# TinfoilHat0/Defending-Against-Backdoors-with-Robust-Learning-Rate

Hardware: NVIDIA H100
Metric: fl_rounds_per_sec (higher is better)
Workload: dtype bf16

## Files before the change

defending-against-backdoors-with-robust-learning-rate_b200/ops/csrc/common.cuh:

```cuda
#pragma once
#include <cuda_runtime.h>
#include <cuda_bf16.h>
#include <stdint.h>

#include "dropspec.h"

#define RLR_CUDA_CHECK(expr)                                                                     \
    do {                                                                                         \
        cudaError_t _e = (expr);                                                                 \
        if (_e != cudaSuccess) return _e;                                                        \
    } while (0)

namespace rlr {

constexpr int kWarp = 32;

__device__ __forceinline__ void pdl_wait() { asm volatile("griddepcontrol.wait;" ::: "memory"); }
__device__ __forceinline__ void pdl_trigger() { asm volatile("griddepcontrol.launch_dependents;" ::: "memory"); }

extern int g_pdl;
bool pdl_enabled();

template <typename... KArgs, typename... Args>
inline cudaError_t launch_kernel(void (*kernel)(KArgs...), dim3 grid, dim3 block, size_t smem, cudaStream_t st, Args&&... args) {
    if (!pdl_enabled()) {
        kernel<<<grid, block, smem, st>>>(static_cast<KArgs>(args)...);
        return cudaGetLastError();
    }
    cudaLaunchConfig_t cfg = {};
    cfg.gridDim = grid; cfg.blockDim = block; cfg.dynamicSmemBytes = smem; cfg.stream = st;
    cudaLaunchAttribute attr[1];
    attr[0].id = cudaLaunchAttributeProgrammaticStreamSerialization;
    attr[0].val.programmaticStreamSerializationAllowed = 1;
    cfg.attrs = attr; cfg.numAttrs = 1;
    return cudaLaunchKernelEx(&cfg, kernel, static_cast<KArgs>(args)...);
}

void* scratch_alloc(size_t bytes, cudaStream_t st);
void scratch_free(void* p);
struct Scratch {
    void* p;
    Scratch(size_t bytes, cudaStream_t st) : p(scratch_alloc(bytes, st)) {}
    ~Scratch() { scratch_free(p); }
    Scratch(const Scratch&) = delete;
    Scratch& operator=(const Scratch&) = delete;
    template <typename T> T* as() const { return static_cast<T*>(p); }
};
template <typename T>
__global__ void __launch_bounds__(256) ordered_sum_kernel(T* __restrict__ out, const T* __restrict__ part, int nparts, long long n) {
    pdl_wait();
    pdl_trigger();
    for (long long i = (long long)blockIdx.x * 256 + threadIdx.x; i < n; i += (long long)gridDim.x * 256) {
        T s = part[i];
        for (int j = 1; j < nparts; ++j) s += part[(size_t)j * n + i];
        out[i] += s;
    }
}

template <typename T>
__global__ void __launch_bounds__(256) ordered_sum_cols_kernel(T* __restrict__ out, const T* __restrict__ part, int nparts, long long n) {
    constexpr int kRows = 64, kPerWarp = kRows / 8;
    __shared__ T tile[kRows][33];
    pdl_wait();
    pdl_trigger();
    const int lane = threadIdx.x & 31, warp = threadIdx.x >> 5;
    const long long col = (long long)blockIdx.x * 32 + lane;
    T s = T(0);
    for (int j0 = 0; j0 < nparts; j0 += kRows) {
        T v[kPerWarp];
#pragma unroll
        for (int q = 0; q < kPerWarp; ++q) {
            const int j = j0 + warp + 8 * q;
            v[q] = (j < nparts && col < n) ? part[(size_t)j * n + col] : T(0);
        }
#pragma unroll
        for (int q = 0; q < kPerWarp; ++q) tile[warp + 8 * q][lane] = v[q];
        __syncthreads();
        if (warp == 0) {
            const int rows = nparts - j0 < kRows ? nparts - j0 : kRows;
            int r = 0;
            if (j0 == 0) { s = tile[0][lane]; r = 1; }
            for (; r < rows; ++r) s += tile[r][lane];
        }
        __syncthreads();
    }
    if (warp == 0 && col < n) out[col] += s;
}

__device__ __forceinline__ unsigned long long gtimer() {
    unsigned long long t;
    asm volatile("mov.u64 %0, %%globaltimer;" : "=l"(t));
    return t;
}

__device__ __forceinline__ float warp_sum(float v) {
#pragma unroll
    for (int o = 16; o > 0; o >>= 1) v += __shfl_xor_sync(0xffffffffu, v, o);
    return v;
}
__device__ __forceinline__ double warp_sum(double v) {
#pragma unroll
    for (int o = 16; o > 0; o >>= 1) v += __shfl_xor_sync(0xffffffffu, v, o);
    return v;
}
__device__ __forceinline__ unsigned long long warp_sum(unsigned long long v) {
#pragma unroll
    for (int o = 16; o > 0; o >>= 1) v += __shfl_xor_sync(0xffffffffu, v, o);
    return v;
}
__device__ __forceinline__ int warp_sum(int v) {
#pragma unroll
    for (int o = 16; o > 0; o >>= 1) v += __shfl_xor_sync(0xffffffffu, v, o);
    return v;
}

__device__ __forceinline__ float warp_transpose_sum32(float (&v)[32], int lane) {
#define RLR_TSTAGE(O, N)                                                         \
    {                                                                            \
        const bool up = (lane & (O)) != 0;                                       \
        _Pragma("unroll") for (int i = 0; i < (N); ++i) {                        \
            const float send = up ? v[i] : v[i + (N)];                           \
            const float keep = up ? v[i + (N)] : v[i];                           \
            v[i] = keep + __shfl_xor_sync(0xffffffffu, send, (O));               \
        }                                                                        \
    }
    RLR_TSTAGE(16, 16) RLR_TSTAGE(8, 8) RLR_TSTAGE(4, 4) RLR_TSTAGE(2, 2) RLR_TSTAGE(1, 1)
#undef RLR_TSTAGE
    return v[0];
}

template <typename T>
__device__ __forceinline__ T block_sum(T v, T* scratch) {
    v = warp_sum(v);
    const int lane = threadIdx.x & 31, wid = threadIdx.x >> 5;
    if (lane == 0) scratch[wid] = v;
    __syncthreads();
    const int nw = (blockDim.x + 31) >> 5;
    v = (threadIdx.x < nw) ? scratch[threadIdx.x] : T(0);
    if (wid == 0) v = warp_sum(v);
    __syncthreads();
    return v;
}

__device__ __forceinline__ float4 ld_stream_f4(const float* p) {
    float4 r;
    asm volatile("ld.global.nc.L1::no_allocate.v4.f32 {%0,%1,%2,%3}, [%4];"
                 : "=f"(r.x), "=f"(r.y), "=f"(r.z), "=f"(r.w) : "l"(p));
    return r;
}
__device__ __forceinline__ float4 ld_f4(const float* p) {
    float4 r;
    asm volatile("ld.global.v4.f32 {%0,%1,%2,%3}, [%4];"
                 : "=f"(r.x), "=f"(r.y), "=f"(r.z), "=f"(r.w) : "l"(p));
    return r;
}
__device__ __forceinline__ float ld_f1(const float* p) {
    float r;
    asm volatile("ld.global.f32 %0, [%1];" : "=f"(r) : "l"(p));
    return r;
}
__device__ __forceinline__ void st_f4(float* p, float4 v) {
    asm volatile("st.global.v4.f32 [%0], {%1,%2,%3,%4};" ::"l"(p), "f"(v.x), "f"(v.y), "f"(v.z), "f"(v.w) : "memory");
}
__device__ __forceinline__ void multimem_st_f4(float* mc, float4 v) {
    asm volatile("multimem.st.relaxed.sys.global.v4.f32 [%0], {%1,%2,%3,%4};" ::"l"(mc), "f"(v.x), "f"(v.y),
                 "f"(v.z), "f"(v.w) : "memory");
}
__device__ __forceinline__ void multimem_st_b2(uint2* mc, uint2 v) {
    asm volatile("multimem.st.relaxed.sys.global.v2.f32 [%0], {%1,%2};" ::"l"(mc), "f"(__uint_as_float(v.x)),
                 "f"(__uint_as_float(v.y)) : "memory");
}

__device__ __forceinline__ void st_release_sys(uint32_t* p, uint32_t v) {
    asm volatile("st.release.sys.global.u32 [%0], %1;" ::"l"(p), "r"(v) : "memory");
}
__device__ __forceinline__ uint32_t ld_acquire_sys(const uint32_t* p) {
    uint32_t v;
    asm volatile("ld.acquire.sys.global.u32 %0, [%1];" : "=r"(v) : "l"(p) : "memory");
    return v;
}
__device__ __forceinline__ void st_release_gpu(uint32_t* p, uint32_t v) {
    asm volatile("st.release.gpu.global.u32 [%0], %1;" ::"l"(p), "r"(v) : "memory");
}
__device__ __forceinline__ uint32_t ld_acquire_gpu(const uint32_t* p) {
    uint32_t v;
    asm volatile("ld.acquire.gpu.global.u32 %0, [%1];" : "=r"(v) : "l"(p) : "memory");
    return v;
}

struct Philox {
    uint32_t k0, k1;
    __device__ __forceinline__ Philox(uint64_t seed) : k0((uint32_t)seed), k1((uint32_t)(seed >> 32)) {}
    __device__ __forceinline__ uint4 operator()(uint64_t ctr, uint64_t stream) const {
        uint32_t c0 = (uint32_t)ctr, c1 = (uint32_t)(ctr >> 32), c2 = (uint32_t)stream, c3 = (uint32_t)(stream >> 32);
        uint32_t a = k0, b = k1;
#pragma unroll
        for (int r = 0; r < 10; ++r) {
            const uint32_t hi0 = __umulhi(0xD2511F53u, c0), lo0 = 0xD2511F53u * c0;
            const uint32_t hi1 = __umulhi(0xCD9E8D57u, c2), lo1 = 0xCD9E8D57u * c2;
            const uint32_t n0 = hi1 ^ c1 ^ a, n2 = hi0 ^ c3 ^ b;
            c0 = n0; c1 = lo1; c2 = n2; c3 = lo0;
            a += 0x9E3779B9u; b += 0xBB67AE85u;
        }
        return make_uint4(c0, c1, c2, c3);
    }
};
__device__ __forceinline__ float u32_to_unit(uint32_t x) {
    return ((float)(x >> 8) + 1.0f) * (1.0f / 16777216.0f);
}
__device__ __forceinline__ float4 philox_normal4(const Philox& ph, uint64_t ctr, uint64_t stream) {
    const uint4 u = ph(ctr, stream);
    const float r0 = sqrtf(-2.0f * logf(u32_to_unit(u.x))), r1 = sqrtf(-2.0f * logf(u32_to_unit(u.z)));
    float s0, c0, s1, c1;
    sincospif(2.0f * u32_to_unit(u.y), &s0, &c0);
    sincospif(2.0f * u32_to_unit(u.w), &s1, &c1);
    return make_float4(r0 * c0, r0 * s0, r1 * c1, r1 * s1);
}

__device__ __forceinline__ uint32_t dropout_keep8(const DropSpec& d, long long q) {
    const Philox ph(d.seed);
    const uint4 u = ph((uint64_t)q, ((uint64_t)(*d.step) << 20) ^ d.stream);
    const uint32_t r[4] = {u.x, u.y, u.z, u.w};
    uint32_t keep = 0;
#pragma unroll
    for (int i = 0; i < 8; ++i) keep |= (uint32_t)(((r[i >> 1] >> (16 * (i & 1))) & 0xffffu) >= d.thr) << i;
    return keep;
}

template <typename T>
inline cudaError_t launch_ordered_sum(T* out, const T* part, int nparts, long long n, cudaStream_t st) {
    if (nparts >= 16)
        return launch_kernel(ordered_sum_cols_kernel<T>, dim3((unsigned)((n + 31) / 32)), dim3(256), (size_t)0, st, out, part, nparts, n);
    long long blocks = (n + 255) / 256;
    if (blocks > 1024) blocks = 1024;
    if (blocks < 1) blocks = 1;
    return launch_kernel(ordered_sum_kernel<T>, dim3((unsigned)blocks), dim3(256), (size_t)0, st, out, part, nparts, n);
}

__device__ __forceinline__ uint32_t pack_bf16x2(float lo, float hi) {
    __nv_bfloat162 v = __floats2bfloat162_rn(lo, hi);
    return *reinterpret_cast<uint32_t*>(&v);
}

}
```

defending-against-backdoors-with-robust-learning-rate_b200/ops/csrc/norm.cu:

```cuda
#include <stdlib.h>

#include "common.cuh"
#include "gemm.h"

namespace rlr {

struct bf8 { float v[8]; };
__device__ __forceinline__ bf8 load8(const __nv_bfloat16* p) {
    const uint4 u = *reinterpret_cast<const uint4*>(p);
    const __nv_bfloat162* h = reinterpret_cast<const __nv_bfloat162*>(&u);
    bf8 r;
#pragma unroll
    for (int i = 0; i < 4; ++i) { const float2 f = __bfloat1622float2(h[i]); r.v[2 * i] = f.x; r.v[2 * i + 1] = f.y; }
    return r;
}
__device__ __forceinline__ void store8(__nv_bfloat16* p, const bf8& r) {
    uint4 u;
    u.x = pack_bf16x2(r.v[0], r.v[1]); u.y = pack_bf16x2(r.v[2], r.v[3]);
    u.z = pack_bf16x2(r.v[4], r.v[5]); u.w = pack_bf16x2(r.v[6], r.v[7]);
    *reinterpret_cast<uint4*>(p) = u;
}
static inline int rows_grid(long long M, int rows_per_block, int num_sms, int per_sm) {
    long long want = (M + rows_per_block - 1) / rows_per_block;
    long long cap = (long long)num_sms * per_sm;
    return (int)(want < 1 ? 1 : (want > cap ? cap : want));
}
static inline bool chan_ok(int C) { return C >= 8 && C <= 2048 && (C % 8) == 0 && (256 % (C / 8)) == 0; }

template <int MODE, bool kRecompute = false>
__global__ void __launch_bounds__(256, MODE == 0 ? 4 : 3) channel_reduce_kernel(const __nv_bfloat16* __restrict__ x, const __nv_bfloat16* __restrict__ dy,
                                                               const __nv_bfloat16* __restrict__ y, const float* __restrict__ mean_rstd,
                                                               float* __restrict__ part , long long M, int C, int relu,
                                                               const float* __restrict__ gamma = nullptr, const float* __restrict__ beta = nullptr,
                                                               int out_cols = 0 ) {
    extern __shared__ float sh[];
    pdl_wait();
    pdl_trigger();
    const int tpr = C / 8, rpi = 256 / tpr;
    const int cg = threadIdx.x % tpr, ry = threadIdx.x / tpr;
    float a[8], b[8], mu[8], rs[8], msc[8], msh[8];
#pragma unroll
    for (int i = 0; i < 8; ++i) { a[i] = 0.f; b[i] = 0.f; mu[i] = 0.f; rs[i] = 1.f; msc[i] = 0.f; msh[i] = 1.f; }
    if (MODE == 1) {
#pragma unroll
        for (int i = 0; i < 8; ++i) { mu[i] = mean_rstd[cg * 8 + i]; rs[i] = mean_rstd[C + cg * 8 + i]; }
        if (kRecompute) {
#pragma unroll
            for (int i = 0; i < 8; ++i) { msc[i] = gamma[cg * 8 + i] * rs[i]; msh[i] = beta[cg * 8 + i] - mu[i] * msc[i]; }
        }
    }
    constexpr int U = MODE == 0 ? 4 : 2;
    const long long stride = (long long)gridDim.x * rpi;
    for (long long r0 = (long long)blockIdx.x * rpi + ry; r0 < M; r0 += stride * U) {
        uint4 xr[U], dr[U], yr[U];
#pragma unroll
        for (int u = 0; u < U; ++u) {
            const long long r = r0 + u * stride;
            const size_t off = (size_t)(r < M ? r : r0) * C + cg * 8;
            xr[u] = *reinterpret_cast<const uint4*>(x + off);
            if (MODE == 1) {
                dr[u] = *reinterpret_cast<const uint4*>(dy + off);
                if (!kRecompute && relu) yr[u] = *reinterpret_cast<const uint4*>(y + off);
            }
        }
#pragma unroll
        for (int u = 0; u < U; ++u) {
            if (r0 + u * stride >= M) continue;
            const __nv_bfloat162* xh = reinterpret_cast<const __nv_bfloat162*>(&xr[u]);
            const __nv_bfloat162* dh = reinterpret_cast<const __nv_bfloat162*>(&dr[u]);
            const __nv_bfloat162* yh = reinterpret_cast<const __nv_bfloat162*>(&yr[u]);
#pragma unroll
            for (int i = 0; i < 4; ++i) {
                const float2 xv = __bfloat1622float2(xh[i]);
                if (MODE == 0) {
                    a[2 * i] += xv.x; a[2 * i + 1] += xv.y; b[2 * i] += xv.x * xv.x; b[2 * i + 1] += xv.y * xv.y;
                } else {
                    float2 dz = __bfloat1622float2(dh[i]);
                    if (!kRecompute && relu) {
                        const float2 yv = __bfloat1622float2(yh[i]);
                        dz.x = yv.x > 0.f ? dz.x : 0.f; dz.y = yv.y > 0.f ? dz.y : 0.f;
                    } else if (kRecompute) {
                        dz.x = (xv.x * msc[2 * i] + msh[2 * i]) > 0.f ? dz.x : 0.f;
                        dz.y = (xv.y * msc[2 * i + 1] + msh[2 * i + 1]) > 0.f ? dz.y : 0.f;
                    }
                    a[2 * i] += dz.x; a[2 * i + 1] += dz.y;
                    b[2 * i] += dz.x * (xv.x - mu[2 * i]) * rs[2 * i]; b[2 * i + 1] += dz.y * (xv.y - mu[2 * i + 1]) * rs[2 * i + 1];
                }
            }
        }
    }
    float* mine = sh + (size_t)ry * 2 * C + cg * 8;
#pragma unroll
    for (int i = 0; i < 8; ++i) { mine[i] = a[i]; mine[C + i] = b[i]; }
    __syncthreads();
    const int ncols = out_cols > 0 ? out_cols : 2 * C;
    float* dst = part + (size_t)blockIdx.x * ncols;
    for (int i = threadIdx.x; i < ncols; i += 256) {
        float t = 0.f;
        for (int r = 0; r < rpi; ++r) t += sh[(size_t)r * 2 * C + i];
        dst[i] = t;
    }
}

cudaError_t launch_ordered_sum_f32(float* out, const float* part, int nparts, long long n, cudaStream_t st) {
    return launch_ordered_sum(out, part, nparts, n, st);
}
cudaError_t launch_ordered_sum_f64(double* out, const double* part, int nparts, long long n, cudaStream_t st) {
    return launch_ordered_sum(out, part, nparts, n, st);
}

cudaError_t launch_channel_stats(const __nv_bfloat16* x, long long M, int C, float* stats, int num_sms, cudaStream_t st, int only_sum, int nslots) {
    if (!chan_ok(C) || nslots < 1) return cudaErrorInvalidValue;
    const int rpi = 256 / (C / 8);
    const int grid = rows_grid(M, rpi * 8, num_sms, nslots >= 4 ? 4 : 2), ncols = only_sum ? C : 2 * C;
    Scratch part((size_t)grid * ncols * sizeof(float), st);
    RLR_CUDA_CHECK(launch_kernel(channel_reduce_kernel<0, false>, dim3(grid), dim3(256), (size_t)rpi * 2 * C * sizeof(float), st, x, nullptr,
                                 nullptr, nullptr, part.as<float>(), M, C, 0, nullptr, nullptr, only_sum ? C : 0));
    return launch_ordered_sum(stats, part.as<float>(), grid, (long long)ncols, st);
}
cudaError_t launch_bn_bwd_reduce(const __nv_bfloat16* dy, const __nv_bfloat16* y, const __nv_bfloat16* x, const float* mean_rstd,
                                 float* dsum, long long M, int C, int relu, int num_sms, cudaStream_t st, const float* gamma,
                                 const float* beta, int nslots) {
    if (!chan_ok(C) || (relu == 2 && (!gamma || !beta)) || (relu == 1 && !y) || nslots < 1) return cudaErrorInvalidValue;
    const int rpi = 256 / (C / 8);
    const int grid = rows_grid(M, rpi * 8, num_sms, nslots >= 3 ? 3 : 2);
    const size_t smem = (size_t)rpi * 2 * C * sizeof(float);
    Scratch part((size_t)grid * 2 * C * sizeof(float), st);
    if (relu == 2)
        RLR_CUDA_CHECK(launch_kernel(channel_reduce_kernel<1, true>, dim3(grid), dim3(256), smem, st, x, dy, y, mean_rstd, part.as<float>(), M, C,
                                     relu, gamma, beta, 0));
    else
        RLR_CUDA_CHECK(launch_kernel(channel_reduce_kernel<1, false>, dim3(grid), dim3(256), smem, st, x, dy, y, mean_rstd, part.as<float>(), M, C,
                                     relu, nullptr, nullptr, 0));
    return launch_ordered_sum(dsum, part.as<float>(), grid, 2LL * C, st);
}

__global__ void bn_finalize_kernel(const float* __restrict__ stats, int slots, float* __restrict__ mean_rstd, float* running_mean,
                                   float* running_var, int C, float count, float eps, float momentum, int train) {
    const int c = blockIdx.x * blockDim.x + threadIdx.x;
    if (c >= C) return;
    if (train) {
        float s1 = 0.f, s2 = 0.f;
        for (int k = 0; k < slots; ++k) { s1 += stats[(size_t)k * 2 * C + c]; s2 += stats[(size_t)k * 2 * C + C + c]; }
        const float mean = s1 / count;
        const float var = fmaxf(s2 / count - mean * mean, 0.f);
        mean_rstd[c] = mean;
        mean_rstd[C + c] = rsqrtf(var + eps);
        running_mean[c] = (1.f - momentum) * running_mean[c] + momentum * mean;
        const float unbiased = count > 1.f ? var * count / (count - 1.f) : var;
        running_var[c] = (1.f - momentum) * running_var[c] + momentum * unbiased;
    } else {
        mean_rstd[c] = running_mean[c];
        mean_rstd[C + c] = rsqrtf(running_var[c] + eps);
    }
}
cudaError_t launch_bn_finalize(const float* stats, int slots, float* mean_rstd, float* running_mean, float* running_var, int C,
                               float count, float eps, float momentum, int train, cudaStream_t st) {
    bn_finalize_kernel<<<(C + 127) / 128, 128, 0, st>>>(stats, slots, mean_rstd, running_mean, running_var, C, count, eps, momentum, train);
    return cudaGetLastError();
}

struct BnFinalize {
    int mode;
    const float* stats; int slots;
    float count, eps, momentum;
    float* running_mean; float* running_var;
};
template <int U, int kMinBlocks>
__global__ void __launch_bounds__(256, kMinBlocks) bn_apply_kernel(const __nv_bfloat16* __restrict__ x, const __nv_bfloat16* __restrict__ res,
                                                         __nv_bfloat16* __restrict__ y, const float* __restrict__ gamma,
                                                         const float* __restrict__ beta, float* __restrict__ mean_rstd,
                                                         long long M, int C, int relu, BnFinalize fin) {
    pdl_wait();
    pdl_trigger();
    const int tpr = C / 8, rpi = 256 / tpr;
    const int cg = threadIdx.x % tpr, ry = threadIdx.x / tpr;
    float sc[8], sh[8];
#pragma unroll
    for (int i = 0; i < 8; ++i) {
        const int c = cg * 8 + i;
        float mean, rstd;
        if (fin.mode == 1) {
            float s1 = 0.f, s2 = 0.f;
            for (int k = 0; k < fin.slots; ++k) { s1 += fin.stats[(size_t)k * 2 * C + c]; s2 += fin.stats[(size_t)k * 2 * C + C + c]; }
            mean = s1 / fin.count;
            const float var = fmaxf(s2 / fin.count - mean * mean, 0.f);
            rstd = rsqrtf(var + fin.eps);
            if (blockIdx.x == 0 && ry == 0) {
                mean_rstd[c] = mean; mean_rstd[C + c] = rstd;
                fin.running_mean[c] = (1.f - fin.momentum) * fin.running_mean[c] + fin.momentum * mean;
                const float unbiased = fin.count > 1.f ? var * fin.count / (fin.count - 1.f) : var;
                fin.running_var[c] = (1.f - fin.momentum) * fin.running_var[c] + fin.momentum * unbiased;
            }
        } else if (fin.mode == 2) {
            mean = fin.running_mean[c]; rstd = rsqrtf(fin.running_var[c] + fin.eps);
        } else {
            mean = mean_rstd[c]; rstd = mean_rstd[C + c];
        }
        sc[i] = gamma[c] * rstd;
        sh[i] = beta[c] - mean * sc[i];
    }
    const long long stride = (long long)gridDim.x * rpi;
    for (long long r0 = (long long)blockIdx.x * rpi + ry; r0 < M; r0 += stride * U) {
        uint4 xr[U], rr[U];
#pragma unroll
        for (int u = 0; u < U; ++u) {
            const long long r = r0 + u * stride;
            const size_t off = (size_t)(r < M ? r : r0) * C + cg * 8;
            xr[u] = *reinterpret_cast<const uint4*>(x + off);
            if (res) rr[u] = *reinterpret_cast<const uint4*>(res + off);
        }
#pragma unroll
        for (int u = 0; u < U; ++u) {
            const long long r = r0 + u * stride;
            if (r >= M) continue;
            const __nv_bfloat162* xh = reinterpret_cast<const __nv_bfloat162*>(&xr[u]);
            const __nv_bfloat162* rh = reinterpret_cast<const __nv_bfloat162*>(&rr[u]);
            bf8 v;
#pragma unroll
            for (int i = 0; i < 4; ++i) {
                const float2 xv = __bfloat1622float2(xh[i]);
                v.v[2 * i] = xv.x * sc[2 * i] + sh[2 * i]; v.v[2 * i + 1] = xv.y * sc[2 * i + 1] + sh[2 * i + 1];
                if (res) { const float2 q = __bfloat1622float2(rh[i]); v.v[2 * i] += q.x; v.v[2 * i + 1] += q.y; }
                if (relu) { v.v[2 * i] = fmaxf(v.v[2 * i], 0.f); v.v[2 * i + 1] = fmaxf(v.v[2 * i + 1], 0.f); }
            }
            store8(y + (size_t)r * C + cg * 8, v);
        }
    }
}
cudaError_t launch_bn_apply(const __nv_bfloat16* x, const __nv_bfloat16* res, __nv_bfloat16* y, const float* gamma, const float* beta,
                            float* mean_rstd, long long M, int C, int relu, int fin_mode, const float* stats, int slots, float count,
                            float eps, float momentum, float* running_mean, float* running_var, int num_sms, cudaStream_t st) {
    if (!chan_ok(C)) return cudaErrorInvalidValue;
    const int rpi = 256 / (C / 8);
    BnFinalize fin{fin_mode, stats, slots, count, eps, momentum, running_mean, running_var};
    static const int unroll = [] { const char* e = getenv("RLR_BN_UNROLL"); return e ? atoi(e) : 1; }();
    static const int occ = [] { const char* e = getenv("RLR_BN_OCC"); return e ? atoi(e) : 0; }();
    if (unroll <= 1 && occ)
        return launch_kernel(bn_apply_kernel<1, 6>, dim3(rows_grid(M, rpi * 4, num_sms, 12)), dim3(256), (size_t)0, st, x, res, y, gamma, beta, mean_rstd,
                             M, C, relu, fin);
    if (unroll <= 1)
        return launch_kernel(bn_apply_kernel<1, 1>, dim3(rows_grid(M, rpi * 4, num_sms, 8)), dim3(256), (size_t)0, st, x, res, y, gamma, beta, mean_rstd, M,
                             C, relu, fin);
    return launch_kernel(bn_apply_kernel<4, 1>, dim3(rows_grid(M, rpi * 4, num_sms, 6)), dim3(256), (size_t)0, st, x, res, y, gamma, beta, mean_rstd, M, C,
                         relu, fin);
}

template <bool kRecompute, int U, int kMinBlocks = 1>
__global__ void __launch_bounds__(256, kMinBlocks) bn_bwd_apply_kernel(const __nv_bfloat16* __restrict__ dy, const __nv_bfloat16* __restrict__ y,
                                                             const __nv_bfloat16* __restrict__ x, const float* __restrict__ gamma,
                                                             const float* __restrict__ mean_rstd, const float* __restrict__ dsum,
                                                             __nv_bfloat16* __restrict__ dx, __nv_bfloat16* __restrict__ dres,
                                                             float* dgamma, float* dbeta, long long M, int C, int relu,
                                                             const float* __restrict__ beta = nullptr, int nslots = 1) {
    pdl_wait();
    pdl_trigger();
    const int tpr = C / 8, rpi = 256 / tpr;
    const int cg = threadIdx.x % tpr, ry = threadIdx.x / tpr;
    float mu[8], rs[8], g[8], k1[8], k2[8], msh[8];
    const float invM = 1.0f / (float)M;
#pragma unroll
    for (int i = 0; i < 8; ++i) {
        const int c = cg * 8 + i;
        mu[i] = mean_rstd[c]; rs[i] = mean_rstd[C + c]; g[i] = gamma[c] * rs[i];
        float s0 = 0.f, s1 = 0.f;
        for (int k = 0; k < nslots; ++k) { s0 += dsum[(size_t)k * 2 * C + c]; s1 += dsum[(size_t)k * 2 * C + C + c]; }
        k1[i] = s0 * invM; k2[i] = s1 * invM;
        msh[i] = kRecompute ? beta[c] - mu[i] * g[i] : 0.f;
    }
    if (blockIdx.x == 0 && ry == 0) {
#pragma unroll
        for (int i = 0; i < 8; ++i) { dbeta[cg * 8 + i] = k1[i] * (float)M; dgamma[cg * 8 + i] = k2[i] * (float)M; }
    }
    const long long stride = (long long)gridDim.x * rpi;
    for (long long r0 = (long long)blockIdx.x * rpi + ry; r0 < M; r0 += stride * U) {
        bf8 dzv[U], xvv[U], yvv[U];
#pragma unroll
        for (int u = 0; u < U; ++u) {
            const long long r = r0 + u * stride;
            const size_t off = (size_t)(r < M ? r : r0) * C + cg * 8;
            dzv[u] = load8(dy + off);
            xvv[u] = load8(x + off);
            if (!kRecompute && relu) yvv[u] = load8(y + off);
        }
#pragma unroll
        for (int u = 0; u < U; ++u) {
            const long long r = r0 + u * stride;
            if (r >= M) continue;
            const size_t off = (size_t)r * C + cg * 8;
            bf8 dz = dzv[u];
            const bf8 xv = xvv[u];
            if (!kRecompute && relu) {
#pragma unroll
                for (int i = 0; i < 8; ++i) dz.v[i] = yvv[u].v[i] > 0.f ? dz.v[i] : 0.f;
            } else if (kRecompute) {
#pragma unroll
                for (int i = 0; i < 8; ++i) dz.v[i] = (xv.v[i] * g[i] + msh[i]) > 0.f ? dz.v[i] : 0.f;
            }
            if (dres) store8(dres + off, dz);
            bf8 o;
#pragma unroll
            for (int i = 0; i < 8; ++i) o.v[i] = g[i] * (dz.v[i] - k1[i] - (xv.v[i] - mu[i]) * rs[i] * k2[i]);
            store8(dx + off, o);
        }
    }
}
cudaError_t launch_bn_bwd_apply(const __nv_bfloat16* dy, const __nv_bfloat16* y, const __nv_bfloat16* x, const float* gamma,
                                const float* mean_rstd, const float* dsum, __nv_bfloat16* dx, __nv_bfloat16* dres, float* dgamma,
                                float* dbeta, long long M, int C, int relu, int num_sms, cudaStream_t st, const float* beta, int nslots) {
    if (!chan_ok(C) || (relu == 2 && !beta) || (relu == 1 && !y) || nslots < 1) return cudaErrorInvalidValue;
    const int rpi = 256 / (C / 8);
    const int grid = rows_grid(M, rpi * 4, num_sms, 8);
    static const int unroll = [] { const char* e = getenv("RLR_BN_UNROLL"); return e ? atoi(e) : 1; }();
    if (unroll > 1) {
        if (relu == 2)
            return launch_kernel(bn_bwd_apply_kernel<true, 2>, dim3(grid), dim3(256), (size_t)0, st, dy, y, x, gamma, mean_rstd, dsum, dx, dres, dgamma,
                                 dbeta, M, C, relu, beta, nslots);
        return launch_kernel(bn_bwd_apply_kernel<false, 2>, dim3(grid), dim3(256), (size_t)0, st, dy, y, x, gamma, mean_rstd, dsum, dx, dres, dgamma, dbeta,
                             M, C, relu, nullptr, nslots);
    }
    static const int occ = [] { const char* e = getenv("RLR_BN_OCC"); return e ? atoi(e) : 0; }();
    if (occ) {
        const int grid2 = rows_grid(M, rpi * 4, num_sms, 12);
        if (relu == 2)
            return launch_kernel(bn_bwd_apply_kernel<true, 1, 4>, dim3(grid2), dim3(256), (size_t)0, st, dy, y, x, gamma, mean_rstd, dsum, dx, dres, dgamma,
                                 dbeta, M, C, relu, beta, nslots);
        return launch_kernel(bn_bwd_apply_kernel<false, 1, 4>, dim3(grid2), dim3(256), (size_t)0, st, dy, y, x, gamma, mean_rstd, dsum, dx, dres, dgamma,
                             dbeta, M, C, relu, nullptr, nslots);
    }
    if (relu == 2)
        return launch_kernel(bn_bwd_apply_kernel<true, 1>, dim3(grid), dim3(256), (size_t)0, st, dy, y, x, gamma, mean_rstd, dsum, dx, dres, dgamma, dbeta, M,
                             C, relu, beta, nslots);
    return launch_kernel(bn_bwd_apply_kernel<false, 1>, dim3(grid), dim3(256), (size_t)0, st, dy, y, x, gamma, mean_rstd, dsum, dx, dres, dgamma, dbeta, M, C,
                         relu, nullptr, nslots);
}

__global__ void __launch_bounds__(256) relu_bwd_kernel(__nv_bfloat16* __restrict__ dy, const __nv_bfloat16* __restrict__ y, long long n8, float scale) {
    for (long long q = (long long)blockIdx.x * blockDim.x + threadIdx.x; q < n8; q += (long long)gridDim.x * blockDim.x) {
        bf8 d = load8(dy + 8 * q);
        const bf8 yv = load8(y + 8 * q);
#pragma unroll
        for (int i = 0; i < 8; ++i) d.v[i] = yv.v[i] > 0.f ? d.v[i] * scale : 0.f;
        store8(dy + 8 * q, d);
    }
}
cudaError_t launch_relu_bwd(__nv_bfloat16* dy, const __nv_bfloat16* y, long long n, int num_sms, cudaStream_t st, float scale) {
    if (n % 8) return cudaErrorInvalidValue;
    relu_bwd_kernel<<<rows_grid(n / 8, 256, num_sms, 8), 256, 0, st>>>(dy, y, n / 8, scale);
    return cudaGetLastError();
}

__global__ void __launch_bounds__(256) maxpool2_fwd_kernel(const __nv_bfloat16* __restrict__ x, __nv_bfloat16* __restrict__ y,
                                                             uint8_t* __restrict__ idx, int B, int H, int W, int C, DropSpec drop) {
    const int Ho = H / 2, Wo = W / 2, cg_n = C / 8;
    const long long total = (long long)B * Ho * Wo * cg_n;
    for (long long t = (long long)blockIdx.x * blockDim.x + threadIdx.x; t < total; t += (long long)gridDim.x * blockDim.x) {
        const int cg = (int)(t % cg_n);
        long long r = t / cg_n;
        const int wo = (int)(r % Wo); r /= Wo;
        const int ho = (int)(r % Ho);
        const int b = (int)(r / Ho);
        const __nv_bfloat16* base = x + (((size_t)b * H + 2 * ho) * W + 2 * wo) * C + cg * 8;
        bf8 best = load8(base);
        uint8_t bi[8] = {0, 0, 0, 0, 0, 0, 0, 0};
#pragma unroll
        for (int k = 1; k < 4; ++k) {
            const bf8 v = load8(base + ((size_t)(k >> 1) * W + (k & 1)) * C);
#pragma unroll
            for (int i = 0; i < 8; ++i) if (v.v[i] > best.v[i]) { best.v[i] = v.v[i]; bi[i] = (uint8_t)k; }
        }
        const size_t o = (((size_t)b * Ho + ho) * Wo + wo) * C + cg * 8;
        if (drop.thr) {
            const uint32_t keep = dropout_keep8(drop, (long long)(o >> 3));
#pragma unroll
            for (int i = 0; i < 8; ++i) best.v[i] = (keep >> i & 1) ? best.v[i] * drop.scale : 0.f;
        }
        store8(y + o, best);
        uint2 pk;
        pk.x = bi[0] | (bi[1] << 8) | (bi[2] << 16) | (bi[3] << 24);
        pk.y = bi[4] | (bi[5] << 8) | (bi[6] << 16) | (bi[7] << 24);
        *reinterpret_cast<uint2*>(idx + o) = pk;
    }
}
__global__ void __launch_bounds__(256) maxpool2_bwd_kernel(const __nv_bfloat16* __restrict__ dy, const uint8_t* __restrict__ idx,
                                                             __nv_bfloat16* __restrict__ dx, const __nv_bfloat16* __restrict__ zmask,
                                                             int B, int H, int W, int C, DropSpec drop) {
    const int Ho = H / 2, Wo = W / 2, cg_n = C / 8;
    const long long total = (long long)B * Ho * Wo * cg_n;
    for (long long t = (long long)blockIdx.x * blockDim.x + threadIdx.x; t < total; t += (long long)gridDim.x * blockDim.x) {
        const int cg = (int)(t % cg_n);
        long long r = t / cg_n;
        const int wo = (int)(r % Wo); r /= Wo;
        const int ho = (int)(r % Ho);
        const int b = (int)(r / Ho);
        const size_t src = (size_t)t * 8;
        bf8 g = load8(dy + src);
        if (drop.thr) {
            const uint32_t keep = dropout_keep8(drop, (long long)(src >> 3));
#pragma unroll
            for (int i = 0; i < 8; ++i) g.v[i] = (keep >> i & 1) ? g.v[i] * drop.scale : 0.f;
        }
        if (zmask) {
            const bf8 z = load8(zmask + src);
#pragma unroll
            for (int i = 0; i < 8; ++i) g.v[i] = z.v[i] > 0.f ? g.v[i] : 0.f;
        }
        const uint2 pk = *reinterpret_cast<const uint2*>(idx + src);
        bf8 zero;
#pragma unroll
        for (int i = 0; i < 8; ++i) zero.v[i] = 0.f;
#pragma unroll
        for (int me = 0; me < 4; ++me) {
            bf8 o;
#pragma unroll
            for (int i = 0; i < 8; ++i) {
                const int k = ((i < 4 ? pk.x : pk.y) >> (8 * (i & 3))) & 0xff;
                o.v[i] = (k == me) ? g.v[i] : 0.f;
            }
            store8(dx + (((size_t)b * H + 2 * ho + (me >> 1)) * W + 2 * wo + (me & 1)) * C + cg * 8, o);
        }
        const bool last_w = (W & 1) && wo == Wo - 1, last_h = (H & 1) && ho == Ho - 1;
        if (last_w) {
            store8(dx + (((size_t)b * H + 2 * ho) * W + W - 1) * C + cg * 8, zero);
            store8(dx + (((size_t)b * H + 2 * ho + 1) * W + W - 1) * C + cg * 8, zero);
        }
        if (last_h) {
            store8(dx + (((size_t)b * H + H - 1) * W + 2 * wo) * C + cg * 8, zero);
            store8(dx + (((size_t)b * H + H - 1) * W + 2 * wo + 1) * C + cg * 8, zero);
            if (last_w) store8(dx + (((size_t)b * H + H - 1) * W + W - 1) * C + cg * 8, zero);
        }
    }
}
static DropSpec make_drop(float p, uint64_t seed, const long long* step, uint64_t stream) {
    DropSpec d{};
    if (p > 0.f && step) { d.thr = (uint32_t)(p * 65536.0f); d.scale = 1.0f / (1.0f - p); d.seed = seed; d.stream = stream; d.step = step; }
    return d;
}
cudaError_t launch_maxpool2_fwd(const __nv_bfloat16* x, __nv_bfloat16* y, uint8_t* idx, int B, int H, int W, int C, cudaStream_t st, float drop_p,
                                uint64_t seed, const long long* step, uint64_t stream) {
    if (C % 8) return cudaErrorInvalidValue;
    const long long total = (long long)B * (H / 2) * (W / 2) * (C / 8);
    maxpool2_fwd_kernel<<<rows_grid(total, 256, 132, 8), 256, 0, st>>>(x, y, idx, B, H, W, C, make_drop(drop_p, seed, step, stream));
    return cudaGetLastError();
}
cudaError_t launch_maxpool2_bwd(const __nv_bfloat16* dy, const uint8_t* idx, __nv_bfloat16* dx, int B, int H, int W, int C, cudaStream_t st, float drop_p,
                                uint64_t seed, const long long* step, uint64_t stream, const __nv_bfloat16* zmask) {
    if (C % 8 || H < 2 || W < 2) return cudaErrorInvalidValue;
    const long long total = (long long)B * (H / 2) * (W / 2) * (C / 8);
    maxpool2_bwd_kernel<<<rows_grid(total, 256, 132, 8), 256, 0, st>>>(dy, idx, dx, zmask, B, H, W, C, make_drop(drop_p, seed, step, stream));
    return cudaGetLastError();
}

__global__ void avgpool_fwd_kernel(const __nv_bfloat16* __restrict__ x, __nv_bfloat16* __restrict__ y, int B, int HW, int C) {
    const int cg_n = C / 8;
    const int t = blockIdx.x * blockDim.x + threadIdx.x;
    if (t >= B * cg_n) return;
    const int b = t / cg_n, cg = t % cg_n;
    float acc[8] = {0, 0, 0, 0, 0, 0, 0, 0};
    for (int p = 0; p < HW; ++p) {
        const bf8 v = load8(x + ((size_t)b * HW + p) * C + cg * 8);
#pragma unroll
        for (int i = 0; i < 8; ++i) acc[i] += v.v[i];
    }
    bf8 o;
#pragma unroll
    for (int i = 0; i < 8; ++i) o.v[i] = acc[i] / (float)HW;
    store8(y + (size_t)b * C + cg * 8, o);
}
__global__ void avgpool_bwd_kernel(const __nv_bfloat16* __restrict__ dy, __nv_bfloat16* __restrict__ dx, int B, int HW, int C) {
    const int cg_n = C / 8;
    const long long t = (long long)blockIdx.x * blockDim.x + threadIdx.x;
    if (t >= (long long)B * HW * cg_n) return;
    const int cg = (int)(t % cg_n);
    const long long bp = t / cg_n;
    const int b = (int)(bp / HW);
    bf8 g = load8(dy + (size_t)b * C + cg * 8);
#pragma unroll
    for (int i = 0; i < 8; ++i) g.v[i] /= (float)HW;
    store8(dx + (size_t)bp * C + cg * 8, g);
}
cudaError_t launch_avgpool_fwd(const __nv_bfloat16* x, __nv_bfloat16* y, int B, int HW, int C, cudaStream_t st) {
    if (C % 8) return cudaErrorInvalidValue;
    avgpool_fwd_kernel<<<(B * (C / 8) + 127) / 128, 128, 0, st>>>(x, y, B, HW, C);
    return cudaGetLastError();
}
cudaError_t launch_avgpool_bwd(const __nv_bfloat16* dy, __nv_bfloat16* dx, int B, int HW, int C, cudaStream_t st) {
// ... 386 lines not shown
```

Baseline: 0.5399.

## Retune batchnorm kernels: reversed tile order, smem constants, narrow ordered-sum kernel

Adds a narrow-column ordered-sum kernel with double-buffered shared-memory tiles for reductions over few columns. The BN stats and backward-reduce kernels now pick unroll depth and CTAs-per-SM from the slot count. The BN apply and backward-apply kernels compute their per-channel constants once per block into shared memory, process row tiles in reverse order (likely to hit rows still in L2 from the preceding pass), and use fixed unroll and occupancy settings in place of the env-var variants. This aims to cut redundant per-thread constant loads, improve cache reuse, and reduce reduction latency, at the cost of an extra __syncthreads and higher register pressure from the larger unrolls.

```diff
diff --git a/defending-against-backdoors-with-robust-learning-rate_b200/ops/csrc/common.cuh b/defending-against-backdoors-with-robust-learning-rate_b200/ops/csrc/common.cuh
--- a/defending-against-backdoors-with-robust-learning-rate_b200/ops/csrc/common.cuh
+++ b/defending-against-backdoors-with-robust-learning-rate_b200/ops/csrc/common.cuh
@@ -87,6 +87,46 @@
     if (warp == 0 && col < n) out[col] += s;
 }
 
+template <typename T>
+__global__ void __launch_bounds__(256) ordered_sum_narrow_kernel(T* __restrict__ out, const T* __restrict__ part, int nparts, long long n) {
+    constexpr int kCols = 8, kRows = 256 * 8 / kCols, kPerThread = kRows * kCols / 256;
+    __shared__ T tile[2][kRows][kCols];
+    pdl_wait();
+    pdl_trigger();
+    const int c = threadIdx.x % kCols, r0 = threadIdx.x / kCols;
+    const long long col = (long long)blockIdx.x * kCols + c;
+    const int nchunks = (nparts + kRows - 1) / kRows;
+    T v[kPerThread];
+    auto load = [&](int chunk) {
+#pragma unroll
+        for (int q = 0; q < kPerThread; ++q) {
+            const int j = chunk * kRows + r0 + (256 / kCols) * q;
+            v[q] = (j < nparts && col < n) ? part[(size_t)j * n + col] : T(0);
+        }
+    };
+    auto stage = [&](int buf) {
+#pragma unroll
+        for (int q = 0; q < kPerThread; ++q) tile[buf][r0 + (256 / kCols) * q][c] = v[q];
+    };
+    load(0);
+    stage(0);
+    __syncthreads();
+    T s = T(0);
+    for (int k = 0; k < nchunks; ++k) {
+        if (k + 1 < nchunks) load(k + 1);
+        if (threadIdx.x < kCols) {
+            const int rows = nparts - k * kRows < kRows ? nparts - k * kRows : kRows;
+            int r = 0;
+            if (k == 0) { s = tile[0][0][threadIdx.x]; r = 1; }
+#pragma unroll 8
+            for (; r < rows; ++r) s += tile[k & 1][r][threadIdx.x];
+        }
+        if (k + 1 < nchunks) stage((k + 1) & 1);
+        __syncthreads();
+    }
+    if (threadIdx.x < kCols && col < n) out[col] += s;
+}
+
 __device__ __forceinline__ unsigned long long gtimer() {
     unsigned long long t;
     asm volatile("mov.u64 %0, %%globaltimer;" : "=l"(t));
@@ -229,6 +269,8 @@
 
 template <typename T>
 inline cudaError_t launch_ordered_sum(T* out, const T* part, int nparts, long long n, cudaStream_t st) {
+    if (nparts >= 16 && n <= 2048)
+        return launch_kernel(ordered_sum_narrow_kernel<T>, dim3((unsigned)((n + 7) / 8)), dim3(256), (size_t)0, st, out, part, nparts, n);
     if (nparts >= 16)
         return launch_kernel(ordered_sum_cols_kernel<T>, dim3((unsigned)((n + 31) / 32)), dim3(256), (size_t)0, st, out, part, nparts, n);
     long long blocks = (n + 255) / 256;
diff --git a/defending-against-backdoors-with-robust-learning-rate_b200/ops/csrc/norm.cu b/defending-against-backdoors-with-robust-learning-rate_b200/ops/csrc/norm.cu
--- a/defending-against-backdoors-with-robust-learning-rate_b200/ops/csrc/norm.cu
+++ b/defending-against-backdoors-with-robust-learning-rate_b200/ops/csrc/norm.cu
@@ -6,14 +6,14 @@
 namespace rlr {
 
 struct bf8 { float v[8]; };
-__device__ __forceinline__ bf8 load8(const __nv_bfloat16* p) {
-    const uint4 u = *reinterpret_cast<const uint4*>(p);
+__device__ __forceinline__ bf8 unpack8(const uint4& u) {
     const __nv_bfloat162* h = reinterpret_cast<const __nv_bfloat162*>(&u);
     bf8 r;
 #pragma unroll
     for (int i = 0; i < 4; ++i) { const float2 f = __bfloat1622float2(h[i]); r.v[2 * i] = f.x; r.v[2 * i + 1] = f.y; }
     return r;
 }
+__device__ __forceinline__ bf8 load8(const __nv_bfloat16* p) { return unpack8(*reinterpret_cast<const uint4*>(p)); }
 __device__ __forceinline__ void store8(__nv_bfloat16* p, const bf8& r) {
     uint4 u;
     u.x = pack_bf16x2(r.v[0], r.v[1]); u.y = pack_bf16x2(r.v[2], r.v[3]);
@@ -27,8 +27,8 @@
 }
 static inline bool chan_ok(int C) { return C >= 8 && C <= 2048 && (C % 8) == 0 && (256 % (C / 8)) == 0; }
 
-template <int MODE, bool kRecompute = false>
-__global__ void __launch_bounds__(256, MODE == 0 ? 4 : 3) channel_reduce_kernel(const __nv_bfloat16* __restrict__ x, const __nv_bfloat16* __restrict__ dy,
+template <int MODE, bool kRecompute, int U, int kCtasPerSm>
+__global__ void __launch_bounds__(256, kCtasPerSm) channel_reduce_kernel(const __nv_bfloat16* __restrict__ x, const __nv_bfloat16* __restrict__ dy,
                                                                const __nv_bfloat16* __restrict__ y, const float* __restrict__ mean_rstd,
                                                                float* __restrict__ part , long long M, int C, int relu,
                                                                const float* __restrict__ gamma = nullptr, const float* __restrict__ beta = nullptr,
@@ -49,7 +49,6 @@
             for (int i = 0; i < 8; ++i) { msc[i] = gamma[cg * 8 + i] * rs[i]; msh[i] = beta[cg * 8 + i] - mu[i] * msc[i]; }
         }
     }
-    constexpr int U = MODE == 0 ? 4 : 2;
     const long long stride = (long long)gridDim.x * rpi;
     for (long long r0 = (long long)blockIdx.x * rpi + ry; r0 < M; r0 += stride * U) {
         uint4 xr[U], dr[U], yr[U];
@@ -114,8 +113,10 @@
     const int rpi = 256 / (C / 8);
     const int grid = rows_grid(M, rpi * 8, num_sms, nslots >= 4 ? 4 : 2), ncols = only_sum ? C : 2 * C;
     Scratch part((size_t)grid * ncols * sizeof(float), st);
-    RLR_CUDA_CHECK(launch_kernel(channel_reduce_kernel<0, false>, dim3(grid), dim3(256), (size_t)rpi * 2 * C * sizeof(float), st, x, nullptr,
-                                 nullptr, nullptr, part.as<float>(), M, C, 0, nullptr, nullptr, only_sum ? C : 0));
+    const size_t smem = (size_t)rpi * 2 * C * sizeof(float);
+    auto kernel = nslots >= 4 ? channel_reduce_kernel<0, false, 4, 4> : channel_reduce_kernel<0, false, 8, 2>;
+    RLR_CUDA_CHECK(launch_kernel(kernel, dim3(grid), dim3(256), smem, st, x, nullptr, nullptr, nullptr, part.as<float>(), M, C, 0, nullptr,
+                                 nullptr, only_sum ? C : 0));
     return launch_ordered_sum(stats, part.as<float>(), grid, (long long)ncols, st);
 }
 cudaError_t launch_bn_bwd_reduce(const __nv_bfloat16* dy, const __nv_bfloat16* y, const __nv_bfloat16* x, const float* mean_rstd,
@@ -123,15 +124,16 @@
                                  const float* beta, int nslots) {
     if (!chan_ok(C) || (relu == 2 && (!gamma || !beta)) || (relu == 1 && !y) || nslots < 1) return cudaErrorInvalidValue;
     const int rpi = 256 / (C / 8);
-    const int grid = rows_grid(M, rpi * 8, num_sms, nslots >= 3 ? 3 : 2);
+    const bool three = nslots >= 3;
+    const int grid = rows_grid(M, rpi * 8, num_sms, three ? 3 : 2);
     const size_t smem = (size_t)rpi * 2 * C * sizeof(float);
     Scratch part((size_t)grid * 2 * C * sizeof(float), st);
     if (relu == 2)
-        RLR_CUDA_CHECK(launch_kernel(channel_reduce_kernel<1, true>, dim3(grid), dim3(256), smem, st, x, dy, y, mean_rstd, part.as<float>(), M, C,
-                                     relu, gamma, beta, 0));
+        RLR_CUDA_CHECK(launch_kernel(three ? channel_reduce_kernel<1, true, 2, 3> : channel_reduce_kernel<1, true, 4, 2>, dim3(grid), dim3(256), smem,
+                                     st, x, dy, y, mean_rstd, part.as<float>(), M, C, relu, gamma, beta, 0));
     else
-        RLR_CUDA_CHECK(launch_kernel(channel_reduce_kernel<1, false>, dim3(grid), dim3(256), smem, st, x, dy, y, mean_rstd, part.as<float>(), M, C,
-                                     relu, nullptr, nullptr, 0));
+        RLR_CUDA_CHECK(launch_kernel(three ? channel_reduce_kernel<1, false, 2, 3> : channel_reduce_kernel<1, false, 4, 2>, dim3(grid), dim3(256), smem,
+                                     st, x, dy, y, mean_rstd, part.as<float>(), M, C, relu, nullptr, nullptr, 0));
     return launch_ordered_sum(dsum, part.as<float>(), grid, 2LL * C, st);
 }
 
@@ -166,19 +168,29 @@
     float count, eps, momentum;
     float* running_mean; float* running_var;
 };
-template <int U, int kMinBlocks>
-__global__ void __launch_bounds__(256, kMinBlocks) bn_apply_kernel(const __nv_bfloat16* __restrict__ x, const __nv_bfloat16* __restrict__ res,
+
+constexpr int kApplyU = 4, kApplyCtasPerSm = 3;
+constexpr int kBwdU = 4, kBwdCtasPerSm = 2;
+
+__device__ __forceinline__ long long rev_tile_row(int t, int nt, int rpi, int ry, long long M, bool& ok) {
+    const long long r = (long long)(nt - 1 - t) * rpi + ry;
+    ok = t < nt && r < M;
+    return r;
+}
+static inline int apply_grid(long long M, int rpi, int U, int num_sms, int per_sm) {
+    const long long nt = (M + rpi - 1) / rpi;
+    return rows_grid(nt, U, num_sms, per_sm);
+}
+
+template <int U>
+__global__ void __launch_bounds__(256, kApplyCtasPerSm) bn_apply_kernel(const __nv_bfloat16* __restrict__ x, const __nv_bfloat16* __restrict__ res,
                                                          __nv_bfloat16* __restrict__ y, const float* __restrict__ gamma,
                                                          const float* __restrict__ beta, float* __restrict__ mean_rstd,
                                                          long long M, int C, int relu, BnFinalize fin) {
+    extern __shared__ float2 apply_cst[];
     pdl_wait();
     pdl_trigger();
-    const int tpr = C / 8, rpi = 256 / tpr;
-    const int cg = threadIdx.x % tpr, ry = threadIdx.x / tpr;
-    float sc[8], sh[8];
-#pragma unroll
-    for (int i = 0; i < 8; ++i) {
-        const int c = cg * 8 + i;
+    for (int c = threadIdx.x; c < C; c += blockDim.x) {
         float mean, rstd;
         if (fin.mode == 1) {
             float s1 = 0.f, s2 = 0.f;
@@ -186,7 +198,7 @@
             mean = s1 / fin.count;
             const float var = fmaxf(s2 / fin.count - mean * mean, 0.f);
             rstd = rsqrtf(var + fin.eps);
-            if (blockIdx.x == 0 && ry == 0) {
+            if (blockIdx.x == 0) {
                 mean_rstd[c] = mean; mean_rstd[C + c] = rstd;
                 fin.running_mean[c] = (1.f - fin.momentum) * fin.running_mean[c] + fin.momentum * mean;
                 const float unbiased = fin.count > 1.f ? var * fin.count / (fin.count - 1.f) : var;
@@ -197,23 +209,33 @@
         } else {
             mean = mean_rstd[c]; rstd = mean_rstd[C + c];
         }
-        sc[i] = gamma[c] * rstd;
-        sh[i] = beta[c] - mean * sc[i];
-    }
-    const long long stride = (long long)gridDim.x * rpi;
-    for (long long r0 = (long long)blockIdx.x * rpi + ry; r0 < M; r0 += stride * U) {
+        const float scale = gamma[c] * rstd;
+        apply_cst[c] = make_float2(scale, beta[c] - mean * scale);
+    }
+    __syncthreads();
+    const int tpr = C / 8, rpi = 256 / tpr;
+    const int cg = threadIdx.x % tpr, ry = threadIdx.x / tpr;
+    float sc[8], sh[8];
+#pragma unroll
+    for (int i = 0; i < 8; ++i) { const float2 k = apply_cst[cg * 8 + i]; sc[i] = k.x; sh[i] = k.y; }
+    const int nt = (int)((M + rpi - 1) / rpi), G = gridDim.x;
+    for (int t0 = blockIdx.x; t0 < nt; t0 += G * U) {
         uint4 xr[U], rr[U];
 #pragma unroll
         for (int u = 0; u < U; ++u) {
-            const long long r = r0 + u * stride;
-            const size_t off = (size_t)(r < M ? r : r0) * C + cg * 8;
-            xr[u] = *reinterpret_cast<const uint4*>(x + off);
-            if (res) rr[u] = *reinterpret_cast<const uint4*>(res + off);
+            bool ok;
+            const long long r = rev_tile_row(t0 + u * G, nt, rpi, ry, M, ok);
+            if (ok) {
+                const size_t off = (size_t)r * C + cg * 8;
+                xr[u] = *reinterpret_cast<const uint4*>(x + off);
+                if (res) rr[u] = *reinterpret_cast<const uint4*>(res + off);
+            }
         }
 #pragma unroll
         for (int u = 0; u < U; ++u) {
-            const long long r = r0 + u * stride;
-            if (r >= M) continue;
+            bool ok;
+            const long long r = rev_tile_row(t0 + u * G, nt, rpi, ry, M, ok);
+            if (!ok) continue;
             const __nv_bfloat162* xh = reinterpret_cast<const __nv_bfloat162*>(&xr[u]);
             const __nv_bfloat162* rh = reinterpret_cast<const __nv_bfloat162*>(&rr[u]);
             bf8 v;
@@ -234,65 +256,67 @@
     if (!chan_ok(C)) return cudaErrorInvalidValue;
     const int rpi = 256 / (C / 8);
     BnFinalize fin{fin_mode, stats, slots, count, eps, momentum, running_mean, running_var};
-    static const int unroll = [] { const char* e = getenv("RLR_BN_UNROLL"); return e ? atoi(e) : 1; }();
-    static const int occ = [] { const char* e = getenv("RLR_BN_OCC"); return e ? atoi(e) : 0; }();
-    if (unroll <= 1 && occ)
-        return launch_kernel(bn_apply_kernel<1, 6>, dim3(rows_grid(M, rpi * 4, num_sms, 12)), dim3(256), (size_t)0, st, x, res, y, gamma, beta, mean_rstd,
-                             M, C, relu, fin);
-    if (unroll <= 1)
-        return launch_kernel(bn_apply_kernel<1, 1>, dim3(rows_grid(M, rpi * 4, num_sms, 8)), dim3(256), (size_t)0, st, x, res, y, gamma, beta, mean_rstd, M,
-                             C, relu, fin);
-    return launch_kernel(bn_apply_kernel<4, 1>, dim3(rows_grid(M, rpi * 4, num_sms, 6)), dim3(256), (size_t)0, st, x, res, y, gamma, beta, mean_rstd, M, C,
-                         relu, fin);
-}
-
-template <bool kRecompute, int U, int kMinBlocks = 1>
-__global__ void __launch_bounds__(256, kMinBlocks) bn_bwd_apply_kernel(const __nv_bfloat16* __restrict__ dy, const __nv_bfloat16* __restrict__ y,
+    return launch_kernel(bn_apply_kernel<kApplyU>, dim3(apply_grid(M, rpi, kApplyU, num_sms, kApplyCtasPerSm)), dim3(256),
+                         (size_t)C * sizeof(float2), st, x, res, y, gamma, beta, mean_rstd, M, C, relu, fin);
+}
+
+template <bool kRecompute, int U>
+__global__ void __launch_bounds__(256, kBwdCtasPerSm) bn_bwd_apply_kernel(const __nv_bfloat16* __restrict__ dy, const __nv_bfloat16* __restrict__ y,
                                                              const __nv_bfloat16* __restrict__ x, const float* __restrict__ gamma,
                                                              const float* __restrict__ mean_rstd, const float* __restrict__ dsum,
                                                              __nv_bfloat16* __restrict__ dx, __nv_bfloat16* __restrict__ dres,
                                                              float* dgamma, float* dbeta, long long M, int C, int relu,
                                                              const float* __restrict__ beta = nullptr, int nslots = 1) {
+    extern __shared__ float bwd_cst[];
     pdl_wait();
     pdl_trigger();
+    const float invM = 1.0f / (float)M;
+    for (int c = threadIdx.x; c < C; c += blockDim.x) {
+        const float mu = mean_rstd[c], rs = mean_rstd[C + c], g = gamma[c] * rs;
+        float s0 = 0.f, s1 = 0.f;
+        for (int k = 0; k < nslots; ++k) { s0 += dsum[(size_t)k * 2 * C + c]; s1 += dsum[(size_t)k * 2 * C + C + c]; }
+        const float k1 = s0 * invM, k2 = s1 * invM;
+        bwd_cst[c] = mu; bwd_cst[C + c] = rs; bwd_cst[2 * C + c] = g; bwd_cst[3 * C + c] = k1; bwd_cst[4 * C + c] = k2;
+        bwd_cst[5 * C + c] = kRecompute ? beta[c] - mu * g : 0.f;
+        if (blockIdx.x == 0) { dbeta[c] = k1 * (float)M; dgamma[c] = k2 * (float)M; }
+    }
+    __syncthreads();
     const int tpr = C / 8, rpi = 256 / tpr;
     const int cg = threadIdx.x % tpr, ry = threadIdx.x / tpr;
     float mu[8], rs[8], g[8], k1[8], k2[8], msh[8];
-    const float invM = 1.0f / (float)M;
 #pragma unroll
     for (int i = 0; i < 8; ++i) {
         const int c = cg * 8 + i;
-        mu[i] = mean_rstd[c]; rs[i] = mean_rstd[C + c]; g[i] = gamma[c] * rs[i];
-        float s0 = 0.f, s1 = 0.f;
-        for (int k = 0; k < nslots; ++k) { s0 += dsum[(size_t)k * 2 * C + c]; s1 += dsum[(size_t)k * 2 * C + C + c]; }
-        k1[i] = s0 * invM; k2[i] = s1 * invM;
-        msh[i] = kRecompute ? beta[c] - mu[i] * g[i] : 0.f;
-    }
-    if (blockIdx.x == 0 && ry == 0) {
-#pragma unroll
-        for (int i = 0; i < 8; ++i) { dbeta[cg * 8 + i] = k1[i] * (float)M; dgamma[cg * 8 + i] = k2[i] * (float)M; }
-    }
-    const long long stride = (long long)gridDim.x * rpi;
-    for (long long r0 = (long long)blockIdx.x * rpi + ry; r0 < M; r0 += stride * U) {
-        bf8 dzv[U], xvv[U], yvv[U];
+        mu[i] = bwd_cst[c]; rs[i] = bwd_cst[C + c]; g[i] = bwd_cst[2 * C + c]; k1[i] = bwd_cst[3 * C + c]; k2[i] = bwd_cst[4 * C + c];
+        msh[i] = bwd_cst[5 * C + c];
+    }
+    const bool need_y = !kRecompute && relu;
+    const int nt = (int)((M + rpi - 1) / rpi), G = gridDim.x;
+    for (int t0 = blockIdx.x; t0 < nt; t0 += G * U) {
+        uint4 dr[U], xr[U], yr[U];
 #pragma unroll
         for (int u = 0; u < U; ++u) {
-            const long long r = r0 + u * stride;
-            const size_t off = (size_t)(r < M ? r : r0) * C + cg * 8;
-            dzv[u] = load8(dy + off);
-            xvv[u] = load8(x + off);
-            if (!kRecompute && relu) yvv[u] = load8(y + off);
+            bool ok;
+            const long long r = rev_tile_row(t0 + u * G, nt, rpi, ry, M, ok);
+            if (ok) {
+                const size_t off = (size_t)r * C + cg * 8;
+                dr[u] = *reinterpret_cast<const uint4*>(dy + off);
+                xr[u] = *reinterpret_cast<const uint4*>(x + off);
+                if (need_y) yr[u] = *reinterpret_cast<const uint4*>(y + off);
+            }
         }
 #pragma unroll
         for (int u = 0; u < U; ++u) {
-            const long long r = r0 + u * stride;
-            if (r >= M) continue;
+            bool ok;
+            const long long r = rev_tile_row(t0 + u * G, nt, rpi, ry, M, ok);
+            if (!ok) continue;
             const size_t off = (size_t)r * C + cg * 8;
-            bf8 dz = dzv[u];
-            const bf8 xv = xvv[u];
-            if (!kRecompute && relu) {
-#pragma unroll
-                for (int i = 0; i < 8; ++i) dz.v[i] = yvv[u].v[i] > 0.f ? dz.v[i] : 0.f;
+            bf8 dz = unpack8(dr[u]);
+            const bf8 xv = unpack8(xr[u]);
+            if (need_y) {
+                const bf8 yv = unpack8(yr[u]);
+#pragma unroll
+                for (int i = 0; i < 8; ++i) dz.v[i] = yv.v[i] > 0.f ? dz.v[i] : 0.f;
             } else if (kRecompute) {
 #pragma unroll
                 for (int i = 0; i < 8; ++i) dz.v[i] = (xv.v[i] * g[i] + msh[i]) > 0.f ? dz.v[i] : 0.f;
@@ -310,28 +334,12 @@
                                 float* dbeta, long long M, int C, int relu, int num_sms, cudaStream_t st, const float* beta, int nslots) {
     if (!chan_ok(C) || (relu == 2 && !beta) || (relu == 1 && !y) || nslots < 1) return cudaErrorInvalidValue;
     const int rpi = 256 / (C / 8);
-    const int grid = rows_grid(M, rpi * 4, num_sms, 8);
-    static const int unroll = [] { const char* e = getenv("RLR_BN_UNROLL"); return e ? atoi(e) : 1; }();
-    if (unroll > 1) {
-        if (relu == 2)
-            return launch_kernel(bn_bwd_apply_kernel<true, 2>, dim3(grid), dim3(256), (size_t)0, st, dy, y, x, gamma, mean_rstd, dsum, dx, dres, dgamma,
-                                 dbeta, M, C, relu, beta, nslots);
-        return launch_kernel(bn_bwd_apply_kernel<false, 2>, dim3(grid), dim3(256), (size_t)0, st, dy, y, x, gamma, mean_rstd, dsum, dx, dres, dgamma, dbeta,
-                             M, C, relu, nullptr, nslots);
-    }
-    static const int occ = [] { const char* e = getenv("RLR_BN_OCC"); return e ? atoi(e) : 0; }();
-    if (occ) {
-        const int grid2 = rows_grid(M, rpi * 4, num_sms, 12);
-        if (relu == 2)
-            return launch_kernel(bn_bwd_apply_kernel<true, 1, 4>, dim3(grid2), dim3(256), (size_t)0, st, dy, y, x, gamma, mean_rstd, dsum, dx, dres, dgamma,
-                                 dbeta, M, C, relu, beta, nslots);
-        return launch_kernel(bn_bwd_apply_kernel<false, 1, 4>, dim3(grid2), dim3(256), (size_t)0, st, dy, y, x, gamma, mean_rstd, dsum, dx, dres, dgamma,
-                             dbeta, M, C, relu, nullptr, nslots);
-    }
+    const dim3 grid(apply_grid(M, rpi, kBwdU, num_sms, kBwdCtasPerSm));
+    const size_t smem = (size_t)6 * C * sizeof(float);
     if (relu == 2)
-        return launch_kernel(bn_bwd_apply_kernel<true, 1>, dim3(grid), dim3(256), (size_t)0, st, dy, y, x, gamma, mean_rstd, dsum, dx, dres, dgamma, dbeta, M,
+        return launch_kernel(bn_bwd_apply_kernel<true, kBwdU>, grid, dim3(256), smem, st, dy, y, x, gamma, mean_rstd, dsum, dx, dres, dgamma, dbeta, M,
                              C, relu, beta, nslots);
-    return launch_kernel(bn_bwd_apply_kernel<false, 1>, dim3(grid), dim3(256), (size_t)0, st, dy, y, x, gamma, mean_rstd, dsum, dx, dres, dgamma, dbeta, M, C,
+    return launch_kernel(bn_bwd_apply_kernel<false, kBwdU>, grid, dim3(256), smem, st, dy, y, x, gamma, mean_rstd, dsum, dx, dres, dgamma, dbeta, M, C,
                          relu, nullptr, nslots);
 }
 
```

New measurement: 0.5837 (median of 6 runs). 1.08x the previous value.
